# peach-xiao/EMRT

Measured on AMD Instinct MI355X. Metric: training tiles/sec at 256x256, higher is better.
Workload: dtype bf16; 1 GPU; EMRT ResNet50, Potsdam 256x256, 6 classes, batch 8 per GPU, fwd+bwd+SGD step (BASELINE configs[1]), bf16; global_batch=8, parallelism=dp1, hipgraph=True

## Files before the change

emrt_amd/csrc/common.hpp:

```cpp
#pragma once
#include <hip/hip_runtime.h>
#include <stdint.h>
#include <stdio.h>
#include <string.h>
#include "../../include/emrt_hip.h"

#define EMRT_F32 0
#define EMRT_BF16 1
#define EMRT_F16 2

namespace emrt {

extern thread_local char g_err[512];
inline int fail(const char* fn, const char* msg) {
  snprintf(g_err, sizeof(g_err), "%s: %s", fn, msg);
  return -1;
}
inline int check_launch(const char* fn) {
  hipError_t e = hipGetLastError();
  if (e != hipSuccess) {
    snprintf(g_err, sizeof(g_err), "%s: launch failed: %s", fn, hipGetErrorString(e));
    return -2;
  }
  return 0;
// ... 7 lines not shown
  int conv_tile;
  int wgrad_split;
  int thin_cblk;
  int thin_blocks;
  int thin_ch;
  int no_thin_bwd;
  int igemm64_nst;
  int wgrad_nst;
  int pair_max;
  int msda_fwd_global;
  int msda_bwd_global;
  int msda_lds_min_pairs;
  int msda_bwd_dref_lds;
  int msda_band_halo;
  int msda_scatter_qsplit;
  int msda_scatter_cuts;
  int msda_fwd_chunks;
  int msda_fwd_threads;
  int msda_fwd_probe;
  int bn_block_kb;
  int bn_operand_blocks;
  int ln_bwd_rows;
  int ln_bwd_max_blocks;
  int ln_bwd_threads;
  int ln_atomic;
  int gn_group_blocks;
  int gn_stat_rows;
  int gn_bwd_stat_rows;
  int gn_apply_rows;
  int igemm8p_probe;
  int igemm8p_cmajor;
  int igemm8p_min_blocks;
  int wgrad8p_min_steps;
  int wgrad8p_slab;
  int wgrad8p_xcd;
  int wgrad8p_force;
  int no_ksplit128;
  int wgrad_no_overwrite;
  int no_s2_dgrad;
  int wgroup_blocks;
  int wgroup_min_steps;
  int wgroup_max;
  int wgroup8;
  int wgroup8_blocks;
  int wgroup8_min_work;
  int msda_scatter_merge;
  int msda_scatter_mfma;
  int msda_mf_bands;
  int sgd_nt;
  int mha_bwd_split;
  int mha_valu;
  int no_bna;
  int memcpy_kernel;
  int xk;
};
extern Tuning g_tune;

struct Scratch {
  void* ptr; size_t bytes; void* stream;
  unsigned* tick;
  float* xk_part;
};
constexpr size_t SCRATCH_TICK_BYTES = 65536;
constexpr int SCRATCH_TICKS = (int)(SCRATCH_TICK_BYTES / 4);
constexpr size_t SCRATCH_XK_BYTES = 8u << 20;
extern Scratch g_scratch;

struct bf16_t {
  unsigned short v;
};
struct f16_t {
  unsigned short v;
};

__device__ __forceinline__ float to_f32(float x) { return x; }
__device__ __forceinline__ float to_f32(bf16_t x) { return __uint_as_float(((uint32_t)x.v) << 16); }
__device__ __forceinline__ float to_f32(f16_t x) { return (float)__builtin_bit_cast(_Float16, x.v); }
__device__ __forceinline__ float bf16_bits_to_f32(uint32_t lo16) { return __uint_as_float(lo16 << 16); }
__device__ __forceinline__ float f16_bits_to_f32(uint32_t lo16) { return (float)__builtin_bit_cast(_Float16, (unsigned short)lo16); }

template <class T>
__device__ __forceinline__ T from_f32(float f);
template <>
__device__ __forceinline__ float from_f32<float>(float f) {
  return f;
}
template <>
__device__ __forceinline__ bf16_t from_f32<bf16_t>(float f) {
  __bf16 b = (__bf16)f;
  bf16_t r;
  r.v = __builtin_bit_cast(unsigned short, b);
  return r;
}
template <>
__device__ __forceinline__ f16_t from_f32<f16_t>(float f) {
  f16_t r;
  r.v = __builtin_bit_cast(unsigned short, (_Float16)f);
  return r;
}
typedef __attribute__((ext_vector_type(2))) _Float16 emrt_half2_t;
typedef __attribute__((ext_vector_type(2))) float emrt_float2_t;
__device__ __forceinline__ uint32_t pack_f16x2(float lo, float hi) {
  emrt_half2_t h = __builtin_convertvector((emrt_float2_t){lo, hi}, emrt_half2_t);
  return __builtin_bit_cast(uint32_t, h);
}
__device__ __forceinline__ void unpack_f16x2(uint32_t w, float& lo, float& hi) {
// ... 216 lines not shown
```

emrt_amd/csrc/elementwise.hip:

```cpp
#include "common.hpp"
#include <stdlib.h>

using namespace emrt;

thread_local char emrt::g_err[512] = {0};

extern "C" const char* emrt_last_error(void) { return emrt::g_err; }
extern "C" int emrt_abi_version(void) { return 9; }

namespace {
struct TuneEntry { const char* name; int emrt::Tuning::*field; int def; };
const TuneEntry kTune[] = {
    {"conv_tile", &emrt::Tuning::conv_tile, 0},         {"wgrad_split", &emrt::Tuning::wgrad_split, 0},
    {"thin_cblk", &emrt::Tuning::thin_cblk, 64},        {"thin_blocks", &emrt::Tuning::thin_blocks, 128},
    {"thin_ch", &emrt::Tuning::thin_ch, 8},             {"no_thin_bwd", &emrt::Tuning::no_thin_bwd, 0},
    {"pair_max", &emrt::Tuning::pair_max, 768},         {"msda_fwd_global", &emrt::Tuning::msda_fwd_global, 0},
    {"bn_block_kb", &emrt::Tuning::bn_block_kb, 8},     {"ln_atomic", &emrt::Tuning::ln_atomic, 1},
    {"msda_fwd_chunks", &emrt::Tuning::msda_fwd_chunks, 0}, {"msda_fwd_threads", &emrt::Tuning::msda_fwd_threads, 1024},
    {"msda_fwd_probe", &emrt::Tuning::msda_fwd_probe, 0}, {"wgrad_nst", &emrt::Tuning::wgrad_nst, 2},
    {"igemm64_nst", &emrt::Tuning::igemm64_nst, 3}, {"msda_bwd_global", &emrt::Tuning::msda_bwd_global, 0},
    {"msda_lds_min_pairs", &emrt::Tuning::msda_lds_min_pairs, 2048}, {"msda_bwd_dref_lds", &emrt::Tuning::msda_bwd_dref_lds, 1},
    {"gn_group_blocks", &emrt::Tuning::gn_group_blocks, 0}, {"gn_stat_rows", &emrt::Tuning::gn_stat_rows, 32},
    {"gn_bwd_stat_rows", &emrt::Tuning::gn_bwd_stat_rows, 32}, {"gn_apply_rows", &emrt::Tuning::gn_apply_rows, 8},
    {"msda_scatter_cuts", &emrt::Tuning::msda_scatter_cuts, 0}, {"msda_scatter_qsplit", &emrt::Tuning::msda_scatter_qsplit, 0}, {"msda_band_halo", &emrt::Tuning::msda_band_halo, 0},
    {"igemm8p_probe", &emrt::Tuning::igemm8p_probe, 0}, {"igemm8p_min_blocks", &emrt::Tuning::igemm8p_min_blocks, 160}, {"igemm8p_cmajor", &emrt::Tuning::igemm8p_cmajor, 0},
    {"wgrad8p_min_steps", &emrt::Tuning::wgrad8p_min_steps, 8}, {"wgrad8p_slab", &emrt::Tuning::wgrad8p_slab, 1}, {"wgrad8p_force", &emrt::Tuning::wgrad8p_force, 0}, {"wgrad8p_xcd", &emrt::Tuning::wgrad8p_xcd, 1},
    {"wgrad_no_overwrite", &emrt::Tuning::wgrad_no_overwrite, 0}, {"no_ksplit128", &emrt::Tuning::no_ksplit128, 0}, {"ln_bwd_rows", &emrt::Tuning::ln_bwd_rows, 0}, {"ln_bwd_max_blocks", &emrt::Tuning::ln_bwd_max_blocks, 0}, {"bn_operand_blocks", &emrt::Tuning::bn_operand_blocks, 0}, {"no_s2_dgrad", &emrt::Tuning::no_s2_dgrad, 0}, {"wgroup_blocks", &emrt::Tuning::wgroup_blocks, 1024}, {"wgroup_min_steps", &emrt::Tuning::wgroup_min_steps, 32}, {"wgroup_max", &emrt::Tuning::wgroup_max, 0},
    {"no_bna", &emrt::Tuning::no_bna, 0}, {"memcpy_kernel", &emrt::Tuning::memcpy_kernel, 0}, {"xk", &emrt::Tuning::xk, 0}, {"mha_valu", &emrt::Tuning::mha_valu, 0}, {"mha_bwd_split", &emrt::Tuning::mha_bwd_split, 1}, {"msda_scatter_merge", &emrt::Tuning::msda_scatter_merge, 0},
    {"wgroup8", &emrt::Tuning::wgroup8, 0}, {"wgroup8_blocks", &emrt::Tuning::wgroup8_blocks, 0}, {"wgroup8_min_work", &emrt::Tuning::wgroup8_min_work, 6000},
    {"msda_scatter_mfma", &emrt::Tuning::msda_scatter_mfma, 1}, {"sgd_nt", &emrt::Tuning::sgd_nt, 1}, {"ln_bwd_threads", &emrt::Tuning::ln_bwd_threads, 512}, {"msda_mf_bands", &emrt::Tuning::msda_mf_bands, 0},
};
emrt::Tuning tuning_from_env() {
  emrt::Tuning t;
  for (const TuneEntry& e : kTune) {
    char env[64] = "EMRT_";
    size_t n = strlen(env);
    for (const char* c = e.name; *c && n + 1 < sizeof(env); ++c) env[n++] = (char)((*c >= 'a' && *c <= 'z') ? *c - 32 : *c);
    env[n] = 0;
    const char* v = (strcmp(e.name, "msda_fwd_probe") == 0 || strcmp(e.name, "igemm8p_probe") == 0) ? nullptr : getenv(env);
    t.*(e.field) = v ? atoi(v) : e.def;
  }
  return t;
}
}
emrt::Tuning emrt::g_tune = tuning_from_env();
emrt::Scratch emrt::g_scratch = {nullptr, 0, nullptr, nullptr, nullptr};

extern "C" int emrt_set_scratch(void* ptr, size_t bytes, void* stream) {
  EMRT_REQUIRE((ptr != nullptr) == (bytes > 0) && ((uintptr_t)ptr) % 256 == 0, "scratch must be 256-byte aligned device memory (or nullptr, 0)");
  if (ptr && ptr == emrt::g_scratch.ptr && emrt::g_scratch.tick && bytes == emrt::g_scratch.bytes + emrt::SCRATCH_TICK_BYTES + emrt::SCRATCH_XK_BYTES) {
    emrt::g_scratch.stream = stream;
    return 0;
  }
  emrt::g_scratch.ptr = ptr;
  emrt::g_scratch.bytes = bytes;
  emrt::g_scratch.stream = stream;
  emrt::g_scratch.tick = nullptr;
  emrt::g_scratch.xk_part = nullptr;
  if (ptr && bytes >= (16u << 20) + emrt::SCRATCH_XK_BYTES + emrt::SCRATCH_TICK_BYTES && bytes % 256 == 0) {
    emrt::g_scratch.bytes = bytes - emrt::SCRATCH_TICK_BYTES - emrt::SCRATCH_XK_BYTES;
    emrt::g_scratch.xk_part = reinterpret_cast<float*>(static_cast<char*>(ptr) + emrt::g_scratch.bytes);
    emrt::g_scratch.tick = reinterpret_cast<unsigned*>(static_cast<char*>(ptr) + emrt::g_scratch.bytes + emrt::SCRATCH_XK_BYTES);
    if (hipMemsetAsync(emrt::g_scratch.tick, 0, emrt::SCRATCH_TICK_BYTES, (hipStream_t)stream) != hipSuccess) {
      emrt::g_scratch.tick = nullptr;
      return emrt::fail("emrt_set_scratch", "cannot zero the arrival counters");
    }
  }
  return 0;
}

extern "C" int emrt_set_tuning(const char* name, int value) {
  EMRT_REQUIRE(name, "null name");
  for (const TuneEntry& e : kTune)
    if (strcmp(e.name, name) == 0) { emrt::g_tune.*(e.field) = value; return 0; }
  return emrt::fail("emrt_set_tuning", "unknown knob");
}
extern "C" int emrt_get_tuning(const char* name, int* value) {
  EMRT_REQUIRE(name && value, "null pointer");
  for (const TuneEntry& e : kTune)
    if (strcmp(e.name, name) == 0) { *value = emrt::g_tune.*(e.field); return 0; }
  return emrt::fail("emrt_get_tuning", "unknown knob");
}

// ... 398 lines not shown
```

emrt_amd/csrc/spatial.hip:

```cpp
#include "common.hpp"
#include "bn_operand.hpp"

using namespace emrt;

struct Axis {
  float s, t;
  int clamp0;
};

__host__ __device__ inline Axis make_axis(int in, int out, int align_corners) {
  Axis a;
  if (align_corners) { a.s = out > 1 ? (float)(in - 1) / (float)(out - 1) : 0.f; a.t = 0.f; a.clamp0 = 0; }
  else { a.s = (float)in / (float)out; a.t = 0.5f * a.s - 0.5f; a.clamp0 = 1; }
  return a;
}

__device__ __forceinline__ void axis_src(const Axis& a, int d, int in, int& i0, int& i1, float& l0, float& l1) {
  float src = a.clamp0 ? a.s * ((float)d + 0.5f) - 0.5f : a.s * (float)d;
  if (a.clamp0 && src < 0.f) src = 0.f;
  i0 = (int)src;
  if (i0 > in - 1) i0 = in - 1;
  i1 = i0 + (i0 < in - 1 ? 1 : 0);
  l1 = src - (float)i0;
  l0 = 1.f - l1;
// ... 63 lines not shown
template <class T, int VEC>
struct ResizeTaps {
  float v00[VEC], v01[VEC], v10[VEC], v11[VEC];
  float wy0, wy1, wx0, wx1;
  long long out_off;
};
template <class T, int VEC>
__device__ __forceinline__ void resize_taps_load(const ResizeArgs& a, long long idx, int cv, bool small, ResizeTaps<T, VEC>& t) {
  int c, ow, oh, n;
  unravel4(idx, cv, a.OW, a.OH, small, c, ow, oh, n);
  c *= VEC;
  int y0, y1, x0, x1;
  axis_src(a.ay, oh, a.IH, y0, y1, t.wy0, t.wy1);
  axis_src(a.ax, ow, a.IW, x0, x1, t.wx0, t.wx1);
  const T* ip = (const T*)a.in + (long long)n * a.in_bs + c;
  VecIO<T, VEC>::load(ip + ((long long)y0 * a.IW + x0) * a.in_ld, t.v00);
  VecIO<T, VEC>::load(ip + ((long long)y0 * a.IW + x1) * a.in_ld, t.v01);
  VecIO<T, VEC>::load(ip + ((long long)y1 * a.IW + x0) * a.in_ld, t.v10);
  VecIO<T, VEC>::load(ip + ((long long)y1 * a.IW + x1) * a.in_ld, t.v11);
  t.out_off = (long long)n * a.out_bs + ((long long)oh * a.OW + ow) * a.out_ld + c;
}
template <class T, int VEC>
__global__ __launch_bounds__(256) void resize_fwd_bn_kernel(ResizeArgs a, BnOperand bn) {
  extern __shared__ float bn_lds[];
  const int cv = a.C / VEC;
  const long long total = (long long)a.N * a.OH * a.OW * cv;
  const bool small = total <= 0xffffffffll;
  const long long step = (long long)gridDim.x * blockDim.x;
  long long idx = (long long)blockIdx.x * blockDim.x + threadIdx.x;
  ResizeTaps<T, VEC> cur, nxt;
  if (idx < total) resize_taps_load<T, VEC>(a, idx, cv, small, cur);
  bn_operand_preamble(bn, a.C, bn_lds, blockIdx.x == 0);
  const float lo = bn.relu ? 0.f : -INFINITY;
  const int c = ((int)threadIdx.x % cv) * VEC;
  float sc[VEC], sh[VEC];
#pragma unroll
  for (int e = 0; e < VEC; ++e) { sc[e] = bn_lds[c + e]; sh[e] = bn_lds[a.C + c + e]; }
  while (idx < total) {
    const long long nidx = idx + step;
    if (nidx < total) resize_taps_load<T, VEC>(a, nidx, cv, small, nxt);
    float o[VEC];
#pragma unroll
    for (int e = 0; e < VEC; ++e) {
      const float t00 = fmaxf(fmaf(cur.v00[e], sc[e], sh[e]), lo), t01 = fmaxf(fmaf(cur.v01[e], sc[e], sh[e]), lo);
      const float t10 = fmaxf(fmaf(cur.v10[e], sc[e], sh[e]), lo), t11 = fmaxf(fmaf(cur.v11[e], sc[e], sh[e]), lo);
      o[e] = cur.wy0 * (cur.wx0 * t00 + cur.wx1 * t01) + cur.wy1 * (cur.wx0 * t10 + cur.wx1 * t11);
    }
    VecIO<T, VEC>::store((T*)a.out + cur.out_off, o);
    cur = nxt;
    idx = nidx;
  }
}

template <class T>
__global__ __launch_bounds__(256) void resize_fwd_nchw_kernel(ResizeArgs a) {
  const long long total = (long long)a.N * a.C * a.OH * a.OW;
  for (long long idx = (long long)blockIdx.x * blockDim.x + threadIdx.x; idx < total; idx += (long long)gridDim.x * blockDim.x) {
    int ow, oh, c, n;
    unravel4(idx, a.OW, a.OH, a.C, total <= 0xffffffffll, ow, oh, c, n);
    int y0, y1, x0, x1;
    float wy0, wy1, wx0, wx1;
    axis_src(a.ay, oh, a.IH, y0, y1, wy0, wy1);
    axis_src(a.ax, ow, a.IW, x0, x1, wx0, wx1);
    const T* ip = (const T*)a.in + (long long)n * a.in_bs + c;
    const float v = wy0 * (wx0 * to_f32(ip[((long long)y0 * a.IW + x0) * a.in_ld]) + wx1 * to_f32(ip[((long long)y0 * a.IW + x1) * a.in_ld])) +
                    wy1 * (wx0 * to_f32(ip[((long long)y1 * a.IW + x0) * a.in_ld]) + wx1 * to_f32(ip[((long long)y1 * a.IW + x1) * a.in_ld]));
    ((float*)a.out)[idx] = v;
  }
}

struct ResizeBwdArgs {
  const void* dout; long long do_bs; int do_ld; int OH, OW;
  void* din; long long di_bs; int di_ld; int IH, IW;
  int N, C;
  Axis ay, ax;
  int dout_nchw_f32;
};

__device__ __forceinline__ void axis_range(const Axis& a, int i, int out, int& lo, int& hi) {
  if (a.s <= 0.f) { lo = 0; hi = out - 1; return; }
  const float t = a.clamp0 ? a.t : 0.f;
  lo = (int)floorf(((float)i - 1.f - t) / a.s);
  hi = (int)ceilf(((float)i + 1.f - t) / a.s);
  if (lo < 0) lo = 0;
  if (hi > out - 1) hi = out - 1;
}

__device__ __forceinline__ float axis_weight(const Axis& a, int d, int in, int i) {
  int i0, i1;
  float l0, l1;
  axis_src(a, d, in, i0, i1, l0, l1);
  return (i0 == i ? l0 : 0.f) + (i1 == i ? l1 : 0.f);
}

constexpr int RB_WIN = 12;

template <class T, int VEC>
__global__ __launch_bounds__(256) void resize_bwd_kernel(ResizeBwdArgs a) {
  const int cv = a.C / VEC;
  const long long total = (long long)a.N * a.IH * a.IW * cv;
  for (long long idx = (long long)blockIdx.x * blockDim.x + threadIdx.x; idx < total; idx += (long long)gridDim.x * blockDim.x) {
    int c, iw, ih, n;
    unravel4(idx, cv, a.IW, a.IH, total <= 0xffffffffll, c, iw, ih, n);
    c *= VEC;
    int ylo, yhi, xlo, xhi;
    axis_range(a.ay, ih, a.OH, ylo, yhi);
    axis_range(a.ax, iw, a.OW, xlo, xhi);
    float acc[VEC];
#pragma unroll
    for (int e = 0; e < VEC; ++e) acc[e] = 0.f;
    const T* gimg = (const T*)a.dout + (long long)n * a.do_bs + c;
    if (xhi - xlo < RB_WIN) {
      float wxa[RB_WIN];
#pragma unroll
      for (int j = 0; j < RB_WIN; ++j) wxa[j] = (xlo + j <= xhi) ? axis_weight(a.ax, xlo + j, a.IW, iw) : 0.f;
      for (int oh = ylo; oh <= yhi; ++oh) {
        const float wy = axis_weight(a.ay, oh, a.IH, ih);
        if (wy == 0.f) continue;
        const T* grow = gimg + ((long long)oh * a.OW + xlo) * a.do_ld;
#pragma unroll
        for (int j = 0; j < RB_WIN; ++j) {
          if (wxa[j] == 0.f) continue;
          const float wgt = wy * wxa[j];
          float g[VEC];
          VecIO<T, VEC>::load(grow + (long long)j * a.do_ld, g);
#pragma unroll
          for (int e = 0; e < VEC; ++e) acc[e] = fmaf(wgt, g[e], acc[e]);
        }
      }
    } else {
      for (int oh = ylo; oh <= yhi; ++oh) {
        const float wy = axis_weight(a.ay, oh, a.IH, ih);
        if (wy == 0.f) continue;
        for (int ow = xlo; ow <= xhi; ++ow) {
          const float wx = axis_weight(a.ax, ow, a.IW, iw);
          if (wx == 0.f) continue;
          const float wgt = wy * wx;
          const T* gp = gimg + ((long long)oh * a.OW + ow) * a.do_ld;
          float g[VEC];
          VecIO<T, VEC>::load(gp, g);
#pragma unroll
          for (int e = 0; e < VEC; ++e) acc[e] = fmaf(wgt, g[e], acc[e]);
        }
      }
    }
    T* dp = (T*)a.din + (long long)n * a.di_bs + ((long long)ih * a.IW + iw) * a.di_ld + c;
    VecIO<T, VEC>::store(dp, acc);
  }
}

constexpr int RBW_THREADS = 1024;
template <class T>
__device__ __forceinline__ void resize_bwd_wide_body(const ResizeBwdArgs& a, const int pixel_block, const int chunk, const int nchunks, float* red) {
  const int iw = pixel_block % a.IW, ih = (pixel_block / a.IW) % a.IH, n = pixel_block / (a.IW * a.IH);
  int ylo, yhi, xlo, xhi;
  axis_range(a.ay, ih, a.OH, ylo, yhi);
  axis_range(a.ax, iw, a.OW, xlo, xhi);
  const int bw = xhi - xlo + 1, npix = (yhi - ylo + 1) * bw;
  const int cq = a.C / 4 / nchunks;
  const int phases = RBW_THREADS / cq;
  const int q = (int)threadIdx.x % cq, ph = (int)threadIdx.x / cq;
  const int qg = chunk * cq + q;
  float acc[4] = {0.f, 0.f, 0.f, 0.f};
  if (ph < phases) {
    const T* gimg = (const T*)a.dout + (long long)n * a.do_bs + qg * 4;
    for (int pxi = ph; pxi < npix; pxi += phases) {
      const int oh = ylo + pxi / bw, ow = xlo + pxi % bw;
      const float wgt = axis_weight(a.ay, oh, a.IH, ih) * axis_weight(a.ax, ow, a.IW, iw);
      if (wgt == 0.f) continue;
      float g[4];
      Vec4<T>::load(gimg + ((long long)oh * a.OW + ow) * a.do_ld, g);
#pragma unroll
      for (int e = 0; e < 4; ++e) acc[e] = fmaf(wgt, g[e], acc[e]);
    }
  }
#pragma unroll
  for (int e = 0; e < 4; ++e) red[threadIdx.x * 4 + e] = acc[e];
  __syncthreads();
  if (ph == 0) {
    for (int o = 1; o < phases; ++o)
#pragma unroll
      for (int e = 0; e < 4; ++e) acc[e] += red[(threadIdx.x + o * cq) * 4 + e];
    Vec4<T>::store((T*)a.din + (long long)n * a.di_bs + ((long long)ih * a.IW + iw) * a.di_ld + qg * 4, acc);
  }
}

template <class T>
__global__ __launch_bounds__(RBW_THREADS) void resize_bwd_wide_kernel(ResizeBwdArgs a) {
  __shared__ float red[RBW_THREADS * 4];
  resize_bwd_wide_body<T>(a, (int)blockIdx.x, (int)blockIdx.y, (int)gridDim.y, red);
}

constexpr int PYR_MAX = 4;
struct PyramidResize {
  ResizeArgs f[PYR_MAX];
  ResizeBwdArgs b[PYR_MAX];
// ... 18 lines not shown
    axis_src(a.ay, oh, a.IH, y0, y1, wy0, wy1);
    axis_src(a.ax, ow, a.IW, x0, x1, wx0, wx1);
    const T* ip = (const T*)a.in + (long long)n * a.in_bs + c;
    float v00[VEC], v01[VEC], v10[VEC], v11[VEC], o[VEC];
    VecIO<T, VEC>::load(ip + ((long long)y0 * a.IW + x0) * a.in_ld, v00);
    VecIO<T, VEC>::load(ip + ((long long)y0 * a.IW + x1) * a.in_ld, v01);
    VecIO<T, VEC>::load(ip + ((long long)y1 * a.IW + x0) * a.in_ld, v10);
    VecIO<T, VEC>::load(ip + ((long long)y1 * a.IW + x1) * a.in_ld, v11);
#pragma unroll
    for (int e = 0; e < VEC; ++e) o[e] = wy0 * (wx0 * v00[e] + wx1 * v01[e]) + wy1 * (wx0 * v10[e] + wx1 * v11[e]);
    VecIO<T, VEC>::store((T*)a.out + (long long)n * a.out_bs + ((long long)oh * a.OW + ow) * a.out_ld + c, o);
  }
}
template <class T>
__global__ __launch_bounds__(RBW_THREADS) void resize_bwd_pyramid_kernel(PyramidResize m) {
  __shared__ float red[RBW_THREADS * 4];
  int s = 0;
  while (s + 1 < m.n && (long long)blockIdx.x >= m.first[s + 1]) ++s;
  const int local = (int)((long long)blockIdx.x - m.first[s]), nch = m.chunks[s];
  resize_bwd_wide_body<T>(m.b[s], local / nch, local % nch, nch, red);
}

__global__ __launch_bounds__(256) void resize_bwd_nchw_w_kernel(ResizeBwdArgs a, float* __restrict__ tmp) {
  const long long total = (long long)a.N * a.C * a.OH * a.IW;
  const float* __restrict__ g = (const float*)a.dout;
  for (long long idx = (long long)blockIdx.x * blockDim.x + threadIdx.x; idx < total; idx += (long long)gridDim.x * blockDim.x) {
    int iw;
    long long row;
    unravel2(idx, a.IW, total <= 0xffffffffll, iw, row);
    int xlo, xhi;
    axis_range(a.ax, iw, a.OW, xlo, xhi);
    const float* gr = g + row * a.OW;
    float acc = 0.f;
    for (int ow = xlo; ow <= xhi; ++ow) acc = fmaf(axis_weight(a.ax, ow, a.IW, iw), gr[ow], acc);
    tmp[idx] = acc;
  }
}

template <class T>
__global__ __launch_bounds__(256) void resize_bwd_nchw_h_kernel(ResizeBwdArgs a, const float* __restrict__ tmp) {
  const long long total = (long long)a.N * a.C * a.IH * a.IW;
  for (long long idx = (long long)blockIdx.x * blockDim.x + threadIdx.x; idx < total; idx += (long long)gridDim.x * blockDim.x) {
    int iw, ih, c, n;
    unravel4(idx, a.IW, a.IH, a.C, total <= 0xffffffffll, iw, ih, c, n);
    int ylo, yhi;
    axis_range(a.ay, ih, a.OH, ylo, yhi);
    const float* tp = tmp + ((long long)n * a.C + c) * a.OH * a.IW + iw;
    float acc = 0.f;
    for (int oh = ylo; oh <= yhi; ++oh) acc = fmaf(axis_weight(a.ay, oh, a.IH, ih), tp[(long long)oh * a.IW], acc);
    ((T*)a.din)[(long long)n * a.di_bs + ((long long)ih * a.IW + iw) * a.di_ld + c] = from_f32<T>(acc);
  }
}

struct PoolArgs {
  const void* in; long long in_bs; int in_ld; int H, W;
  void* out; long long out_bs; int out_ld;
  int N, C, nscales;
  int k[4], tok0[4];
  int ntok;
  int parts[4], item0[4], nitem;
};

__device__ __forceinline__ void bin_of(int i, int k, int S, int& b0, int& b1) {
  b0 = (i * S) / k;
  b1 = ((i + 1) * S + k - 1) / k;
}

constexpr int POOL_THREADS = 1024;

template <class T>
__global__ __launch_bounds__(POOL_THREADS) void adaptive_pool_fwd_kernel(PoolArgs a) {
  __shared__ float red[POOL_THREADS * 4];
  const int tok = blockIdx.x % a.ntok, n = blockIdx.x / a.ntok;
  int s = 0;
  while (s + 1 < a.nscales && tok >= a.tok0[s + 1]) ++s;
  const int k = a.k[s], t = tok - a.tok0[s];
  const int oi = t / k, oj = t - oi * k;
  int h0, h1, w0, w1;
  bin_of(oi, k, a.H, h0, h1);
  bin_of(oj, k, a.W, w0, w1);
  const int bw = w1 - w0, npix = (h1 - h0) * bw;
  const int cq = (a.C + 3) / 4;
  int phases = POOL_THREADS / cq;
  if (phases < 1) phases = 1;
  const bool vec = (a.C % 4 == 0) && (a.in_ld % 4 == 0) && (a.in_bs % 4 == 0) && (((uintptr_t)a.in) % 16 == 0);
  const float inv = 1.f / (float)npix;
  for (int q0 = 0; q0 < cq; q0 += POOL_THREADS) {
    const int q = q0 + (int)threadIdx.x % (cq < POOL_THREADS ? cq : POOL_THREADS);
    const int ph = (int)threadIdx.x / (cq < POOL_THREADS ? cq : POOL_THREADS);
    float acc[4] = {0.f, 0.f, 0.f, 0.f};
    if (q < cq && ph < phases) {
      const T* ip = (const T*)a.in + (long long)n * a.in_bs + q * 4;
      if (vec) {
        constexpr int U = 8;
        for (int px0 = ph; px0 < npix; px0 += phases * U) {
          float v[U][4];
#pragma unroll
          for (int u = 0; u < U; ++u) {
            const int pxi = px0 + u * phases;
            const int pc = pxi < npix ? pxi : ph;
            const int hh = h0 + pc / bw, ww = w0 + pc % bw;
            Vec4<T>::load(ip + ((long long)hh * a.W + ww) * a.in_ld, v[u]);
          }
#pragma unroll
          for (int u = 0; u < U; ++u) {
            const bool ok = px0 + u * phases < npix;
// ... 295 lines not shown
  }
}

template <class T>
__global__ __launch_bounds__(256) void nchw_to_nhwc_kernel(const float* __restrict__ in, T* __restrict__ out, int N, int C, int H, int W, int CO) {
  const long long total = (long long)N * H * W * CO;
  for (long long idx = (long long)blockIdx.x * blockDim.x + threadIdx.x; idx < total; idx += (long long)gridDim.x * blockDim.x) {
    int c, w, h, n;
    unravel4(idx, CO, W, H, total <= 0xffffffffll, c, w, h, n);
    out[idx] = from_f32<T>(c < C ? in[(((long long)n * C + c) * H + h) * W + w] : 0.f);
  }
}

template <class T, int CO>
__global__ __launch_bounds__(256) void nchw_to_nhwc_pix_kernel(const float* __restrict__ in, T* __restrict__ out, int N, int C, long long HW) {
  const long long total = (long long)N * HW;
  for (long long idx = (long long)blockIdx.x * blockDim.x + threadIdx.x; idx < total; idx += (long long)gridDim.x * blockDim.x) {
    long long n, p;
    if (total <= 0xffffffffll) { const unsigned q = (unsigned)idx / (unsigned)HW; n = q; p = (unsigned)idx - q * (unsigned)HW; }
    else { n = idx / HW; p = idx - n * HW; }
    float v[CO];
#pragma unroll
    for (int c = 0; c < CO; ++c) v[c] = c < C ? in[(n * C + c) * HW + p] : 0.f;
    if constexpr (CO == 8) Vec8<T>::store(out + idx * 8, v);
    else Vec4<T>::store(out + idx * 4, v);
  }
}

static inline int ew_grid(long long total) {
  long long g = (total + 255) / 256;
  if (g > 8192) g = 8192;
  if (g < 1) g = 1;
  return (int)g;
}

extern "C" int emrt_resize_bilinear_fwd(const void* in, long long in_bs, int in_ld, int IH, int IW, void* out, long long out_bs,
                                        int out_ld, int OH, int OW, const void* add, long long add_bs, int add_ld, int N, int C,
                                        int align_corners, int out_nchw_f32, int dtype, void* stream) {
  EMRT_REQUIRE_FWD_DTYPE(dtype);
  EMRT_REQUIRE(in && out, "null pointer");
  EMRT_REQUIRE(N > 0 && C > 0 && IH > 0 && IW > 0 && OH > 0 && OW > 0, "bad dims");
  EMRT_REQUIRE(!(out_nchw_f32 && add), "addend not supported with NCHW output");
  ResizeArgs a;
  a.in = in; a.in_bs = in_bs; a.in_ld = in_ld; a.IH = IH; a.IW = IW;
  a.out = out; a.out_bs = out_bs; a.out_ld = out_ld; a.OH = OH; a.OW = OW;
  a.add = add; a.add_bs = add_bs; a.add_ld = add_ld; a.N = N; a.C = C;
  a.ay = make_axis(IH, OH, align_corners); a.ax = make_axis(IW, OW, align_corners); a.out_nchw_f32 = out_nchw_f32;
  hipStream_t st = (hipStream_t)stream;
  const bool v4 = C % 4 == 0 && in_ld % 4 == 0 && out_ld % 4 == 0 && in_bs % 4 == 0 && out_bs % 4 == 0 &&
                  (!add || (add_ld % 4 == 0 && add_bs % 4 == 0)) && ((uintptr_t)in % 16 == 0) && ((uintptr_t)out % 16 == 0) &&
                  (!add || (uintptr_t)add % 16 == 0);
  const bool v8 = v4 && dtype != EMRT_F32 && C % 8 == 0 && in_ld % 8 == 0 && out_ld % 8 == 0 && in_bs % 8 == 0 && out_bs % 8 == 0 &&
                  (!add || (add_ld % 8 == 0 && add_bs % 8 == 0));
  return with_fwd_dtype("emrt_resize_bilinear_fwd", dtype, [&](auto t) {
    using T = decltype(t);
    if (out_nchw_f32) {
      const int grid = ew_grid((long long)N * C * OH * OW);
      hipLaunchKernelGGL((resize_fwd_nchw_kernel<T>), dim3(grid), dim3(256), 0, st, a);
    } else if (v8) {
      const int grid = ew_grid((long long)N * OH * OW * (C / 8));
      if constexpr (sizeof(T) == 2) hipLaunchKernelGGL((resize_fwd_kernel<T, 8>), dim3(grid), dim3(256), 0, st, a);
    } else if (v4) {
      const int grid = ew_grid((long long)N * OH * OW * (C / 4));
      hipLaunchKernelGGL((resize_fwd_kernel<T, 4>), dim3(grid), dim3(256), 0, st, a);
    } else {
      const int grid = ew_grid((long long)N * OH * OW * C);
      hipLaunchKernelGGL((resize_fwd_kernel<T, 1>), dim3(grid), dim3(256), 0, st, a);
    }
    return check_launch("emrt_resize_bilinear_fwd");
  });
}

static inline int bn_operand_grid(long long total) {
  const int g = ew_grid(total);
  const int cap = g_tune.bn_operand_blocks > 0 ? g_tune.bn_operand_blocks : 1024;
  return g > cap ? cap : g;
}

static int fill_bn_operand(BnOperand& b, const double* sums, double count, float eps, float momentum, float* mean, float* invstd,
                           float* run_mean, float* run_var, const float* gamma, const float* beta, int relu) {
  if (!sums || !mean || !invstd || !gamma || !beta || !(count > 0.0) || (run_mean != nullptr) != (run_var != nullptr)) return -1;
  b.sums = sums; b.inv_count = 1.0 / count; b.eps = eps; b.momentum = momentum; b.mean = mean; b.invstd = invstd;
  b.run_mean = run_mean; b.run_var = run_var; b.gamma = gamma; b.beta = beta; b.relu = relu;
  return 0;
}

extern "C" int emrt_bn_resize_bilinear_fwd(const void* in, long long in_bs, int in_ld, int IH, int IW, void* out, long long out_bs,
                                           int out_ld, int OH, int OW, int N, int C, int align_corners, const double* sums, double count,
                                           float eps, float momentum, float* mean, float* invstd, float* run_mean, float* run_var,
                                           const float* gamma, const float* beta, int relu, int dtype, void* stream) {
  EMRT_REQUIRE_TRAIN_DTYPE(dtype);
  EMRT_REQUIRE(in && out, "null pointer");
  EMRT_REQUIRE(N > 0 && C > 0 && IH > 0 && IW > 0 && OH > 0 && OW > 0, "bad dims");
  ResizeArgs a;
  a.in = in; a.in_bs = in_bs; a.in_ld = in_ld; a.IH = IH; a.IW = IW;
  a.out = out; a.out_bs = out_bs; a.out_ld = out_ld; a.OH = OH; a.OW = OW;
  a.add = nullptr; a.add_bs = 0; a.add_ld = 0; a.N = N; a.C = C;
  a.ay = make_axis(IH, OH, align_corners); a.ax = make_axis(IW, OW, align_corners); a.out_nchw_f32 = 0;
  BnOperand b;
  EMRT_REQUIRE(fill_bn_operand(b, sums, count, eps, momentum, mean, invstd, run_mean, run_var, gamma, beta, relu) == 0,
               "BatchNorm operand: sums, mean, invstd, gamma, beta and a positive count are required");
  const bool v4 = C % 4 == 0 && C <= 1024 && 256 % (C / 4) == 0 && in_ld % 4 == 0 && out_ld % 4 == 0 && in_bs % 4 == 0 && out_bs % 4 == 0 &&
                  ((uintptr_t)in % 16 == 0) && ((uintptr_t)out % 16 == 0);
  EMRT_REQUIRE(v4, "vector path only: C / 4 a divisor of 256, 16-byte aligned rows");
  const bool v8 = dtype != EMRT_F32 && C % 8 == 0 && 256 % (C / 8) == 0 && in_ld % 8 == 0 && out_ld % 8 == 0 && in_bs % 8 == 0 && out_bs % 8 == 0;
  hipStream_t st = (hipStream_t)stream;
  const size_t lds = (size_t)2 * C * sizeof(float);
  return with_train_dtype("emrt_bn_resize_bilinear_fwd", dtype, [&](auto t) {
    using T = decltype(t);
    if (v8) {
      if constexpr (sizeof(T) == 2) hipLaunchKernelGGL((resize_fwd_bn_kernel<T, 8>), dim3(bn_operand_grid((long long)N * OH * OW * (C / 8))), dim3(256), lds, st, a, b);
    } else hipLaunchKernelGGL((resize_fwd_bn_kernel<T, 4>), dim3(bn_operand_grid((long long)N * OH * OW * (C / 4))), dim3(256), lds, st, a, b);
    return check_launch("emrt_bn_resize_bilinear_fwd");
  });
}

extern "C" size_t emrt_resize_bwd_workspace_bytes(int N, int C, int OH, int IW, int dout_nchw_f32) {
  return dout_nchw_f32 ? (size_t)N * C * OH * IW * sizeof(float) : 0;
}

extern "C" int emrt_resize_bilinear_bwd(const void* dout, long long do_bs, int do_ld, int OH, int OW, void* din, long long di_bs,
                                        int di_ld, int IH, int IW, int N, int C, int align_corners, int dout_nchw_f32,
                                        void* workspace, int dtype, void* stream) {
  EMRT_REQUIRE_TRAIN_DTYPE(dtype);
  EMRT_REQUIRE(dout && din, "null pointer");
  ResizeBwdArgs a;
  a.dout = dout; a.do_bs = do_bs; a.do_ld = do_ld; a.OH = OH; a.OW = OW;
  a.din = din; a.di_bs = di_bs; a.di_ld = di_ld; a.IH = IH; a.IW = IW; a.N = N; a.C = C;
  a.ay = make_axis(IH, OH, align_corners); a.ax = make_axis(IW, OW, align_corners); a.dout_nchw_f32 = dout_nchw_f32;
  hipStream_t st = (hipStream_t)stream;
  if (dout_nchw_f32) EMRT_REQUIRE(workspace, "fp32 NCHW gradient needs the emrt_resize_bwd_workspace_bytes() workspace");
  const bool v4 = C % 4 == 0 && do_ld % 4 == 0 && di_ld % 4 == 0 && do_bs % 4 == 0 && di_bs % 4 == 0 &&
                  ((uintptr_t)dout % 16 == 0) && ((uintptr_t)din % 16 == 0);
  const bool v8 = v4 && dtype != EMRT_F32 && C % 8 == 0 && do_ld % 8 == 0 && di_ld % 8 == 0 && do_bs % 8 == 0 && di_bs % 8 == 0;
  return with_train_dtype("emrt_resize_bilinear_bwd", dtype, [&](auto t) {
    using T = decltype(t);
    if (dout_nchw_f32) {
      float* tmp = (float*)workspace;
      hipLaunchKernelGGL(resize_bwd_nchw_w_kernel, dim3(ew_grid((long long)N * C * OH * IW)), dim3(256), 0, st, a, tmp);
      const int grid = ew_grid((long long)N * C * IH * IW);
      hipLaunchKernelGGL((resize_bwd_nchw_h_kernel<T>), dim3(grid), dim3(256), 0, st, a, (const float*)tmp);
    } else if (v4 && C / 4 <= RBW_THREADS && ((long long)OH * OW >= 16ll * IH * IW)) {
      int chunks = 1;
      while (chunks < 8 && (long long)N * IH * IW * chunks < 256 && (C / 4) % (chunks * 2) == 0 && (C / 4) / (chunks * 2) >= 8) chunks *= 2;
      const dim3 grid((unsigned)(N * IH * IW), (unsigned)chunks);
      hipLaunchKernelGGL((resize_bwd_wide_kernel<T>), grid, dim3(RBW_THREADS), 0, st, a);
    } else if (v8) {
      const int grid = ew_grid((long long)N * IH * IW * (C / 8));
      if constexpr (sizeof(T) == 2) hipLaunchKernelGGL((resize_bwd_kernel<T, 8>), dim3(grid), dim3(256), 0, st, a);
    } else if (v4) {
      const int grid = ew_grid((long long)N * IH * IW * (C / 4));
      hipLaunchKernelGGL((resize_bwd_kernel<T, 4>), dim3(grid), dim3(256), 0, st, a);
    } else {
      const int grid = ew_grid((long long)N * IH * IW * C);
      hipLaunchKernelGGL((resize_bwd_kernel<T, 1>), dim3(grid), dim3(256), 0, st, a);
    }
    return check_launch("emrt_resize_bilinear_bwd");
  });
}

static int pyramid_fill(PyramidResize& m, const void* tokens, const int* scales, int nscales, void* const* maps, const int* ld, const long long* bs,
                        int OH, int OW, int N, int C, int align_corners, int esz) {
  if (!tokens || !scales || !maps || !ld || !bs || nscales < 1 || nscales > PYR_MAX || N <= 0 || C <= 0 || OH <= 0 || OW <= 0) return -1;
  if (C % 4 || ((uintptr_t)tokens % 16)) return -2;
  int ntok = 0;
  for (int i = 0; i < nscales; ++i) ntok += scales[i] * scales[i];
  int start = 0;
  m.n = nscales;
  for (int i = 0; i < nscales; ++i) {
    const int k = scales[i];
    if (k <= 0 || !maps[i] || ld[i] % 4 || bs[i] % 4 || ((uintptr_t)maps[i] % 16)) return -2;
    const char* tk = (const char*)tokens + (size_t)start * C * esz;
    ResizeArgs& f = m.f[i];
    f.in = tk; f.in_bs = (long long)ntok * C; f.in_ld = C; f.IH = k; f.IW = k;
    f.out = maps[i]; f.out_bs = bs[i]; f.out_ld = ld[i]; f.OH = OH; f.OW = OW;
    f.add = nullptr; f.add_bs = 0; f.add_ld = 0; f.N = N; f.C = C;
    f.ay = make_axis(k, OH, align_corners); f.ax = make_axis(k, OW, align_corners); f.out_nchw_f32 = 0;
    ResizeBwdArgs& b = m.b[i];
    b.dout = maps[i]; b.do_bs = bs[i]; b.do_ld = ld[i]; b.OH = OH; b.OW = OW;
    b.din = const_cast<char*>(tk); b.di_bs = (long long)ntok * C; b.di_ld = C; b.IH = k; b.IW = k; b.N = N; b.C = C;
    b.ay = f.ay; b.ax = f.ax; b.dout_nchw_f32 = 0;
    start += k * k;
  }
  return 0;
}

extern "C" int emrt_pyramid_resize_fwd(const void* tokens, const int* scales, int nscales, void* const* outs, const int* out_ld,
                                       const long long* out_bs, int OH, int OW, int N, int C, int align_corners, int dtype, void* stream) {
  EMRT_REQUIRE_FWD_DTYPE(dtype);
  PyramidResize m;
  const int rc = pyramid_fill(m, tokens, scales, nscales, outs, out_ld, out_bs, OH, OW, N, C, align_corners, dtype == EMRT_F32 ? 4 : 2);
  EMRT_REQUIRE(rc != -1, "null pointer or bad dims (1..4 scales)");
  EMRT_REQUIRE(rc == 0, "vector path only: C % 4 == 0, 16-byte aligned rows");
  const bool v8 = dtype != EMRT_F32 && C % 8 == 0;
  bool all8 = v8;
  for (int i = 0; i < nscales; ++i) all8 = all8 && out_ld[i] % 8 == 0 && out_bs[i] % 8 == 0;
  const int vec = all8 ? 8 : 4;
  m.first[0] = 0;
  for (int i = 0; i < nscales; ++i) m.first[i + 1] = m.first[i] + (long long)N * OH * OW * (C / vec);
  EMRT_REQUIRE(m.first[nscales] <= 0xffffffffll, "too many elements");
  hipStream_t st = (hipStream_t)stream;
  const int grid = ew_grid(m.first[nscales]);
  return with_fwd_dtype("emrt_pyramid_resize_fwd", dtype, [&](auto t) {
    using T = decltype(t);
// ... 450 lines not shown
```

Baseline: 1009 tiles/s.

## Add specialized bilinear resize kernels for exact 2x upsampling and NCHW paths

Adds a 2x-upsample forward kernel that computes four output pixels per input tap quad using fixed 0.25/0.75 weights, with an optional fused BN+ReLU variant. Adds a 2x backward kernel that gathers a fixed 4x4 neighbourhood. Also adds a 4-wide vectorized NCHW fp32 forward kernel and a fused LDS-based NCHW backward kernel that replaces the two-pass workspace approach. All of these are gated by a new head_stream tuning flag that is on by default. The aim is to cut the index arithmetic, redundant tap loads and extra kernel launches in the segmentation head's resize ops. In exchange the code has more dispatch branches, and the fused backward kernel's LDS use limits occupancy.

New measurement: 1016 tiles/s (median of 6 runs). About the same (+0.7%).

```diff
diff --git a/emrt_amd/csrc/common.hpp b/emrt_amd/csrc/common.hpp
--- a/emrt_amd/csrc/common.hpp
+++ b/emrt_amd/csrc/common.hpp
@@ -83,6 +83,7 @@
   int mha_valu;
   int no_bna;
   int memcpy_kernel;
+  int head_stream;
   int xk;
 };
 extern Tuning g_tune;
diff --git a/emrt_amd/csrc/elementwise.hip b/emrt_amd/csrc/elementwise.hip
--- a/emrt_amd/csrc/elementwise.hip
+++ b/emrt_amd/csrc/elementwise.hip
@@ -29,6 +29,7 @@
     {"no_bna", &emrt::Tuning::no_bna, 0}, {"memcpy_kernel", &emrt::Tuning::memcpy_kernel, 0}, {"xk", &emrt::Tuning::xk, 0}, {"mha_valu", &emrt::Tuning::mha_valu, 0}, {"mha_bwd_split", &emrt::Tuning::mha_bwd_split, 1}, {"msda_scatter_merge", &emrt::Tuning::msda_scatter_merge, 0},
     {"wgroup8", &emrt::Tuning::wgroup8, 0}, {"wgroup8_blocks", &emrt::Tuning::wgroup8_blocks, 0}, {"wgroup8_min_work", &emrt::Tuning::wgroup8_min_work, 6000},
     {"msda_scatter_mfma", &emrt::Tuning::msda_scatter_mfma, 1}, {"sgd_nt", &emrt::Tuning::sgd_nt, 1}, {"ln_bwd_threads", &emrt::Tuning::ln_bwd_threads, 512}, {"msda_mf_bands", &emrt::Tuning::msda_mf_bands, 0},
+    {"head_stream", &emrt::Tuning::head_stream, 1},
 };
 emrt::Tuning tuning_from_env() {
   emrt::Tuning t;
diff --git a/emrt_amd/csrc/spatial.hip b/emrt_amd/csrc/spatial.hip
--- a/emrt_amd/csrc/spatial.hip
+++ b/emrt_amd/csrc/spatial.hip
@@ -139,6 +139,87 @@
   }
 }
 
+__device__ __forceinline__ void x2_axis(int p, int in, int& i0, int& i1, float& b0, float& b1) {
+  i0 = p > 0 ? p - 1 : 0;
+  i1 = i0 + (i0 < in - 1 ? 1 : 0);
+  b0 = p > 0 ? 0.25f : 1.f;
+  b1 = p > 0 ? 0.75f : 0.f;
+}
+template <int VEC>
+struct X2Taps {
+  float v00[VEC], v01[VEC], v10[VEC], v11[VEC];
+  float by0, by1, bx0, bx1;
+  long long out_off;
+  bool ya, yb, xa, xb;
+};
+template <class T, int VEC>
+__device__ __forceinline__ void x2_taps_load(const ResizeArgs& a, unsigned q, int c, X2Taps<VEC>& t) {
+  const unsigned PW = (unsigned)a.IW + 1u, PH = (unsigned)a.IH + 1u;
+  unsigned r = q / PW;
+  const int px = (int)(q - r * PW);
+  const unsigned n = r / PH;
+  const int py = (int)(r - n * PH);
+  int y0, y1, x0, x1;
+  x2_axis(py, a.IH, y0, y1, t.by0, t.by1);
+  x2_axis(px, a.IW, x0, x1, t.bx0, t.bx1);
+  const T* ip = (const T*)a.in + (long long)n * a.in_bs + c;
+  VecIO<T, VEC>::load(ip + (y0 * a.IW + x0) * a.in_ld, t.v00);
+  VecIO<T, VEC>::load(ip + (y0 * a.IW + x1) * a.in_ld, t.v01);
+  VecIO<T, VEC>::load(ip + (y1 * a.IW + x0) * a.in_ld, t.v10);
+  VecIO<T, VEC>::load(ip + (y1 * a.IW + x1) * a.in_ld, t.v11);
+  t.ya = py > 0; t.yb = py < a.IH; t.xa = px > 0; t.xb = px < a.IW;
+  t.out_off = (long long)n * a.out_bs + (long long)((2 * py - 1) * a.OW + 2 * px - 1) * a.out_ld + c;
+}
+template <class T, int VEC, bool BN>
+__global__ __launch_bounds__(256) void resize_fwd_x2_kernel(ResizeArgs a, BnOperand bn) {
+  extern __shared__ float bn_lds[];
+  const int cv = a.C / VEC, ppb = 256 / cv;
+  const unsigned total = (unsigned)a.N * ((unsigned)a.IH + 1u) * ((unsigned)a.IW + 1u);
+  const unsigned step = gridDim.x * (unsigned)ppb;
+  const int c = ((int)threadIdx.x % cv) * VEC;
+  unsigned q = blockIdx.x * (unsigned)ppb + threadIdx.x / (unsigned)cv;
+  X2Taps<VEC> cur, nxt;
+  if (q < total) x2_taps_load<T, VEC>(a, q, c, cur);
+  float sc[VEC], sh[VEC];
+  float lo = -INFINITY;
+  if constexpr (BN) {
+    bn_operand_preamble(bn, a.C, bn_lds, blockIdx.x == 0);
+    lo = bn.relu ? 0.f : -INFINITY;
+#pragma unroll
+    for (int e = 0; e < VEC; ++e) { sc[e] = bn_lds[c + e]; sh[e] = bn_lds[a.C + c + e]; }
+  }
+  const long long row = (long long)a.OW * a.out_ld;
+  while (q < total) {
+    const unsigned nq = q + step;
+    if (nq < total) x2_taps_load<T, VEC>(a, nq, c, nxt);
+    float oaa[VEC], oab[VEC], oba[VEC], obb[VEC];
+#pragma unroll
+    for (int e = 0; e < VEC; ++e) {
+      float t00 = cur.v00[e], t01 = cur.v01[e], t10 = cur.v10[e], t11 = cur.v11[e];
+      if constexpr (BN) {
+        t00 = fmaxf(fmaf(t00, sc[e], sh[e]), lo); t01 = fmaxf(fmaf(t01, sc[e], sh[e]), lo);
+        t10 = fmaxf(fmaf(t10, sc[e], sh[e]), lo); t11 = fmaxf(fmaf(t11, sc[e], sh[e]), lo);
+      }
+      const float ay0 = 0.75f, ay1 = 0.25f, ax0 = 0.75f, ax1 = 0.25f;
+      oaa[e] = ay0 * (ax0 * t00 + ax1 * t01) + ay1 * (ax0 * t10 + ax1 * t11);
+      oab[e] = ay0 * (cur.bx0 * t00 + cur.bx1 * t01) + ay1 * (cur.bx0 * t10 + cur.bx1 * t11);
+      oba[e] = cur.by0 * (ax0 * t00 + ax1 * t01) + cur.by1 * (ax0 * t10 + ax1 * t11);
+      obb[e] = cur.by0 * (cur.bx0 * t00 + cur.bx1 * t01) + cur.by1 * (cur.bx0 * t10 + cur.bx1 * t11);
+    }
+    T* op = (T*)a.out + cur.out_off;
+    if (cur.ya && cur.xa) VecIO<T, VEC>::store(op, oaa);
+    if (cur.ya && cur.xb) VecIO<T, VEC>::store(op + a.out_ld, oab);
+    if (cur.yb && cur.xa) VecIO<T, VEC>::store(op + row, oba);
+    if (cur.yb && cur.xb) VecIO<T, VEC>::store(op + row + a.out_ld, obb);
+    cur = nxt;
+    q = nq;
+  }
+}
+static inline bool resize_x2_geometry(int IH, int IW, int OH, int OW, int N, int in_ld, int out_ld, int align_corners) {
+  return g_tune.head_stream != 0 && !align_corners && OH == 2 * IH && OW == 2 * IW && (long long)N * (IH + 1) * (IW + 1) < 0x7fffffffll &&
+         (long long)IH * IW * in_ld < 0x7fffffffll && (long long)OH * OW < 0x7fffffffll;
+}
+
 template <class T>
 __global__ __launch_bounds__(256) void resize_fwd_nchw_kernel(ResizeArgs a) {
   const long long total = (long long)a.N * a.C * a.OH * a.OW;
@@ -156,6 +237,40 @@
   }
 }
 
+template <class T>
+__global__ __launch_bounds__(256) void resize_fwd_nchw4_kernel(ResizeArgs a) {
+  const int OWq = (a.OW + 3) >> 2;
+  const unsigned total = (unsigned)a.N * a.C * a.OH * OWq;
+  const bool vec = (a.OW & 3) == 0;
+  for (unsigned idx = blockIdx.x * blockDim.x + threadIdx.x; idx < total; idx += gridDim.x * blockDim.x) {
+    int q, oh, c, n;
+    unravel4((long long)idx, OWq, a.OH, a.C, true, q, oh, c, n);
+    int y0, y1;
+    float wy0, wy1;
+    axis_src(a.ay, oh, a.IH, y0, y1, wy0, wy1);
+    const T* ip = (const T*)a.in + (long long)n * a.in_bs + c;
+    const T* r0 = ip + y0 * a.IW * a.in_ld;
+    const T* r1 = ip + y1 * a.IW * a.in_ld;
+    float o[4];
+#pragma unroll
+    for (int e = 0; e < 4; ++e) {
+      const int ow = min(4 * q + e, a.OW - 1);
+      int x0, x1;
+      float wx0, wx1;
+      axis_src(a.ax, ow, a.IW, x0, x1, wx0, wx1);
+      o[e] = wy0 * (wx0 * to_f32(r0[x0 * a.in_ld]) + wx1 * to_f32(r0[x1 * a.in_ld])) +
+             wy1 * (wx0 * to_f32(r1[x0 * a.in_ld]) + wx1 * to_f32(r1[x1 * a.in_ld]));
+    }
+    float* op = (float*)a.out + (((long long)n * a.C + c) * a.OH + oh) * a.OW + 4 * q;
+    if (vec) *reinterpret_cast<float4*>(op) = make_float4(o[0], o[1], o[2], o[3]);
+    else {
+#pragma unroll
+      for (int e = 0; e < 4; ++e)
+        if (4 * q + e < a.OW) op[e] = o[e];
+    }
+  }
+}
+
 struct ResizeBwdArgs {
   const void* dout; long long do_bs; int do_ld; int OH, OW;
   void* din; long long di_bs; int di_ld; int IH, IW;
@@ -164,7 +279,7 @@
   int dout_nchw_f32;
 };
 
-__device__ __forceinline__ void axis_range(const Axis& a, int i, int out, int& lo, int& hi) {
+__host__ __device__ __forceinline__ void axis_range(const Axis& a, int i, int out, int& lo, int& hi) {
   if (a.s <= 0.f) { lo = 0; hi = out - 1; return; }
   const float t = a.clamp0 ? a.t : 0.f;
   lo = (int)floorf(((float)i - 1.f - t) / a.s);
@@ -229,6 +344,61 @@
 #pragma unroll
           for (int e = 0; e < VEC; ++e) acc[e] = fmaf(wgt, g[e], acc[e]);
         }
+      }
+    }
+    T* dp = (T*)a.din + (long long)n * a.di_bs + ((long long)ih * a.IW + iw) * a.di_ld + c;
+    VecIO<T, VEC>::store(dp, acc);
+  }
+}
+
+__device__ __forceinline__ void x2_bwd_axis(int i, int in, float (&w)[4]) {
+  w[0] = i > 0 ? 0.25f : 0.f;
+  w[1] = i > 0 ? 0.75f : 1.f;
+  w[2] = i < in - 1 ? 0.75f : 1.f;
+  w[3] = i < in - 1 ? 0.25f : 0.f;
+}
+template <class T, int VEC>
+__device__ __forceinline__ void unpack16(const uint4& r, float (&o)[VEC]) {
+  if constexpr (sizeof(T) == 4) { o[0] = __uint_as_float(r.x); o[1] = __uint_as_float(r.y); o[2] = __uint_as_float(r.z); o[3] = __uint_as_float(r.w); }
+  else Vec8<T>::unpack(r, o);
+}
+template <class T, int VEC>
+__global__ __launch_bounds__(256) void resize_bwd_x2_kernel(ResizeBwdArgs a) {
+  static_assert(VEC * sizeof(T) == 16, "16-byte vectors");
+  const int cv = a.C / VEC;
+  const unsigned total = (unsigned)a.N * a.IH * a.IW * cv;
+  for (unsigned idx = blockIdx.x * blockDim.x + threadIdx.x; idx < total; idx += gridDim.x * blockDim.x) {
+    int c, iw, ih, n;
+    unravel4((long long)idx, cv, a.IW, a.IH, true, c, iw, ih, n);
+    c *= VEC;
+    float wy[4], wx[4];
+    x2_bwd_axis(ih, a.IH, wy);
+    x2_bwd_axis(iw, a.IW, wx);
+    const T* gimg = (const T*)a.dout + (long long)n * a.do_bs + c;
+    uint4 raw[4][4];
+#pragma unroll
+    for (int j = 0; j < 4; ++j) {
+      const int oh = min(max(2 * ih - 1 + j, 0), a.OH - 1);
+#pragma unroll
+      for (int i = 0; i < 4; ++i) {
+        const int ow = min(max(2 * iw - 1 + i, 0), a.OW - 1);
+        raw[j][i] = *reinterpret_cast<const uint4*>(gimg + (oh * a.OW + ow) * a.do_ld);
+      }
+    }
+    float acc[VEC];
+#pragma unroll
+    for (int e = 0; e < VEC; ++e) acc[e] = 0.f;
+#pragma unroll
+    for (int j = 0; j < 4; ++j) {
+      if (wy[j] == 0.f) continue;
+#pragma unroll
+      for (int i = 0; i < 4; ++i) {
+        if (wx[i] == 0.f) continue;
+        const float wgt = wy[j] * wx[i];
+        float g[VEC];
+        unpack16<T, VEC>(raw[j][i], g);
+#pragma unroll
+        for (int e = 0; e < VEC; ++e) acc[e] = fmaf(wgt, g[e], acc[e]);
       }
     }
     T* dp = (T*)a.din + (long long)n * a.di_bs + ((long long)ih * a.IW + iw) * a.di_ld + c;
@@ -353,6 +523,84 @@
   }
 }
 
+struct NchwBwdPlan { int rh, max_rows; size_t lds; };
+template <class T>
+__global__ __launch_bounds__(256) void resize_bwd_nchw_fused_kernel(ResizeBwdArgs a, int rh, int max_rows) {
+  extern __shared__ float4 nb_lds[];
+  float4* tab = nb_lds;
+  float* rows = reinterpret_cast<float*>(tab + a.OW);
+  float* tmp = rows + (size_t)max_rows * (a.OW + 1);
+  const int tid = threadIdx.x, RS = a.OW + 1, TS = a.IW + 1;
+  const int nbh = (a.IH + rh - 1) / rh;
+  const int plane = (int)blockIdx.x / nbh, bh = (int)blockIdx.x - plane * nbh;
+  const int ih0 = bh * rh, ih1 = min(ih0 + rh, a.IH);
+  int ylo, yhi, unused;
+  axis_range(a.ay, ih0, a.OH, ylo, unused);
+  axis_range(a.ay, ih1 - 1, a.OH, unused, yhi);
+  const int nrows = min(yhi - ylo + 1, max_rows);
+  const float* __restrict__ g = (const float*)a.dout + ((long long)plane * a.OH + ylo) * a.OW;
+  if ((a.OW & 3) == 0) {
+    const int ow4 = a.OW >> 2;
+    for (int it = tid; it < nrows * ow4; it += 256) {
+      const int r = it / ow4, q = it - r * ow4;
+      const float4 v = *reinterpret_cast<const float4*>(g + (long long)it * 4);
+      float* d = rows + r * RS + q * 4;
+      d[0] = v.x; d[1] = v.y; d[2] = v.z; d[3] = v.w;
+    }
+  } else {
+    for (int it = tid; it < nrows * a.OW; it += 256) {
+      const int r = it / a.OW;
+      rows[r * RS + it - r * a.OW] = g[it];
+    }
+  }
+  for (int ow = tid; ow < a.OW; ow += 256) {
+    int x0, x1;
+    float l0, l1;
+    axis_src(a.ax, ow, a.IW, x0, x1, l0, l1);
+    tab[ow] = make_float4(__int_as_float(x0), __int_as_float(x1), l0, l1);
+  }
+  __syncthreads();
+  for (int it = tid; it < nrows * a.IW; it += 256) {
+    const int iw = it / nrows, r = it - iw * nrows;
+    int xlo, xhi;
+    axis_range(a.ax, iw, a.OW, xlo, xhi);
+    const float* gr = rows + r * RS;
+    float acc = 0.f;
+    for (int ow = xlo; ow <= xhi; ++ow) {
+      const float4 t = tab[ow];
+      const float w = (__float_as_int(t.x) == iw ? t.z : 0.f) + (__float_as_int(t.y) == iw ? t.w : 0.f);
+      acc = fmaf(w, gr[ow], acc);
+    }
+    tmp[r * TS + iw] = acc;
+  }
+  __syncthreads();
+  const int n = plane / a.C, c = plane - n * a.C;
+  for (int it = tid; it < (ih1 - ih0) * a.IW; it += 256) {
+    const int j = it / a.IW, iw = it - j * a.IW, ih = ih0 + j;
+    int lo, hi;
+    axis_range(a.ay, ih, a.OH, lo, hi);
+    float acc = 0.f;
+    for (int oh = lo; oh <= hi; ++oh) acc = fmaf(axis_weight(a.ay, oh, a.IH, ih), tmp[(oh - ylo) * TS + iw], acc);
+    ((T*)a.din)[(long long)n * a.di_bs + ((long long)ih * a.IW + iw) * a.di_ld + c] = from_f32<T>(acc);
+  }
+}
+static inline bool nchw_bwd_plan(const ResizeBwdArgs& a, NchwBwdPlan& p) {
+  if (g_tune.head_stream == 0 || (long long)a.N * a.C * a.IH >= 0x7fffffffll || (long long)a.OH * a.OW >= 0x7fffffffll || (uintptr_t)a.dout % 16) return false;
+  for (int rh = 8; rh >= 1; rh >>= 1) {
+    int rows = 0;
+    for (int ih0 = 0; ih0 < a.IH; ih0 += rh) {
+      int ylo, yhi, unused;
+      axis_range(a.ay, ih0, a.OH, ylo, unused);
+      axis_range(a.ay, (ih0 + rh < a.IH ? ih0 + rh : a.IH) - 1, a.OH, unused, yhi);
+      if (yhi - ylo + 1 > rows) rows = yhi - ylo + 1;
+    }
+    const size_t lds = (size_t)a.OW * 16 + (size_t)rows * (a.OW + 1 + a.IW + 1) * sizeof(float);
+    const long long blocks = (long long)a.N * a.C * ((a.IH + rh - 1) / rh);
+    if (lds <= 48 * 1024 && (blocks >= 512 || rh == 1)) { p.rh = rh; p.max_rows = rows; p.lds = lds; return true; }
+  }
+  return false;
+}
+
 struct PoolArgs {
   const void* in; long long in_bs; int in_ld; int H, W;
   void* out; long long out_bs; int out_ld;
@@ -754,17 +1002,24 @@
                   (!add || (uintptr_t)add % 16 == 0);
   const bool v8 = v4 && dtype != EMRT_F32 && C % 8 == 0 && in_ld % 8 == 0 && out_ld % 8 == 0 && in_bs % 8 == 0 && out_bs % 8 == 0 &&
                   (!add || (add_ld % 8 == 0 && add_bs % 8 == 0));
+  const bool x2 = !add && resize_x2_geometry(IH, IW, OH, OW, N, in_ld, out_ld, align_corners);
   return with_fwd_dtype("emrt_resize_bilinear_fwd", dtype, [&](auto t) {
     using T = decltype(t);
     if (out_nchw_f32) {
-      const int grid = ew_grid((long long)N * C * OH * OW);
-      hipLaunchKernelGGL((resize_fwd_nchw_kernel<T>), dim3(grid), dim3(256), 0, st, a);
+      const long long quads = (long long)N * C * OH * ((OW + 3) / 4);
+      if (g_tune.head_stream != 0 && quads < 0x7fffffffll && (long long)IH * IW * in_ld < 0x7fffffffll && (uintptr_t)out % 16 == 0)
+        hipLaunchKernelGGL((resize_fwd_nchw4_kernel<T>), dim3(ew_grid(quads)), dim3(256), 0, st, a);
+      else hipLaunchKernelGGL((resize_fwd_nchw_kernel<T>), dim3(ew_grid((long long)N * C * OH * OW)), dim3(256), 0, st, a);
     } else if (v8) {
       const int grid = ew_grid((long long)N * OH * OW * (C / 8));
-      if constexpr (sizeof(T) == 2) hipLaunchKernelGGL((resize_fwd_kernel<T, 8>), dim3(grid), dim3(256), 0, st, a);
+      if constexpr (sizeof(T) == 2) {
+        if (x2 && 256 % (C / 8) == 0) hipLaunchKernelGGL((resize_fwd_x2_kernel<T, 8, false>), dim3(ew_grid((long long)N * (IH + 1) * (IW + 1) * (C / 8))), dim3(256), 0, st, a, BnOperand{});
+        else hipLaunchKernelGGL((resize_fwd_kernel<T, 8>), dim3(grid), dim3(256), 0, st, a);
+      }
     } else if (v4) {
       const int grid = ew_grid((long long)N * OH * OW * (C / 4));
-      hipLaunchKernelGGL((resize_fwd_kernel<T, 4>), dim3(grid), dim3(256), 0, st, a);
+      if (x2 && C / 4 <= 256 && 256 % (C / 4) == 0) hipLaunchKernelGGL((resize_fwd_x2_kernel<T, 4, false>), dim3(ew_grid((long long)N * (IH + 1) * (IW + 1) * (C / 4))), dim3(256), 0, st, a, BnOperand{});
+      else hipLaunchKernelGGL((resize_fwd_kernel<T, 4>), dim3(grid), dim3(256), 0, st, a);
     } else {
       const int grid = ew_grid((long long)N * OH * OW * C);
       hipLaunchKernelGGL((resize_fwd_kernel<T, 1>), dim3(grid), dim3(256), 0, st, a);
@@ -810,9 +1065,14 @@
   const size_t lds = (size_t)2 * C * sizeof(float);
   return with_train_dtype("emrt_bn_resize_bilinear_fwd", dtype, [&](auto t) {
     using T = decltype(t);
+    const bool x2 = resize_x2_geometry(IH, IW, OH, OW, N, in_ld, out_ld, align_corners);
     if (v8) {
-      if constexpr (sizeof(T) == 2) hipLaunchKernelGGL((resize_fwd_bn_kernel<T, 8>), dim3(bn_operand_grid((long long)N * OH * OW * (C / 8))), dim3(256), lds, st, a, b);
-    } else hipLaunchKernelGGL((resize_fwd_bn_kernel<T, 4>), dim3(bn_operand_grid((long long)N * OH * OW * (C / 4))), dim3(256), lds, st, a, b);
+      if constexpr (sizeof(T) == 2) {
+        if (x2) hipLaunchKernelGGL((resize_fwd_x2_kernel<T, 8, true>), dim3(bn_operand_grid((long long)N * (IH + 1) * (IW + 1) * (C / 8))), dim3(256), lds, st, a, b);
+        else hipLaunchKernelGGL((resize_fwd_bn_kernel<T, 8>), dim3(bn_operand_grid((long long)N * OH * OW * (C / 8))), dim3(256), lds, st, a, b);
+      }
+    } else if (x2) hipLaunchKernelGGL((resize_fwd_x2_kernel<T, 4, true>), dim3(bn_operand_grid((long long)N * (IH + 1) * (IW + 1) * (C / 4))), dim3(256), lds, st, a, b);
+    else hipLaunchKernelGGL((resize_fwd_bn_kernel<T, 4>), dim3(bn_operand_grid((long long)N * OH * OW * (C / 4))), dim3(256), lds, st, a, b);
     return check_launch("emrt_bn_resize_bilinear_fwd");
   });
 }
@@ -835,9 +1095,16 @@
   const bool v4 = C % 4 == 0 && do_ld % 4 == 0 && di_ld % 4 == 0 && do_bs % 4 == 0 && di_bs % 4 == 0 &&
                   ((uintptr_t)dout % 16 == 0) && ((uintptr_t)din % 16 == 0);
   const bool v8 = v4 && dtype != EMRT_F32 && C % 8 == 0 && do_ld % 8 == 0 && di_ld % 8 == 0 && do_bs % 8 == 0 && di_bs % 8 == 0;
+  const bool x2 = g_tune.head_stream != 0 && !align_corners && OH == 2 * IH && OW == 2 * IW && (long long)OH * OW * do_ld < 0x7fffffffll &&
+                  (long long)N * IH * IW * C < 0x7fffffffll;
   return with_train_dtype("emrt_resize_bilinear_bwd", dtype, [&](auto t) {
     using T = decltype(t);
     if (dout_nchw_f32) {
+      NchwBwdPlan pl;
+      if (nchw_bwd_plan(a, pl)) {
+        hipLaunchKernelGGL((resize_bwd_nchw_fused_kernel<T>), dim3((unsigned)(N * C * ((IH + pl.rh - 1) / pl.rh))), dim3(256), pl.lds, st, a, pl.rh, pl.max_rows);
+        return check_launch("emrt_resize_bilinear_bwd");
+      }
       float* tmp = (float*)workspace;
       hipLaunchKernelGGL(resize_bwd_nchw_w_kernel, dim3(ew_grid((long long)N * C * OH * IW)), dim3(256), 0, st, a, tmp);
       const int grid = ew_grid((long long)N * C * IH * IW);
@@ -849,9 +1116,15 @@
       hipLaunchKernelGGL((resize_bwd_wide_kernel<T>), grid, dim3(RBW_THREADS), 0, st, a);
     } else if (v8) {
       const int grid = ew_grid((long long)N * IH * IW * (C / 8));
-      if constexpr (sizeof(T) == 2) hipLaunchKernelGGL((resize_bwd_kernel<T, 8>), dim3(grid), dim3(256), 0, st, a);
+      if constexpr (sizeof(T) == 2) {
+        if (x2) hipLaunchKernelGGL((resize_bwd_x2_kernel<T, 8>), dim3(grid), dim3(256), 0, st, a);
+        else hipLaunchKernelGGL((resize_bwd_kernel<T, 8>), dim3(grid), dim3(256), 0, st, a);
+      }
     } else if (v4) {
       const int grid = ew_grid((long long)N * IH * IW * (C / 4));
+      if constexpr (sizeof(T) == 4) {
+        if (x2) { hipLaunchKernelGGL((resize_bwd_x2_kernel<T, 4>), dim3(grid), dim3(256), 0, st, a); return check_launch("emrt_resize_bilinear_bwd"); }
+      }
       hipLaunchKernelGGL((resize_bwd_kernel<T, 4>), dim3(grid), dim3(256), 0, st, a);
     } else {
       const int grid = ew_grid((long long)N * IH * IW * C);
```
